# 13Karl/CUDA-Image-and-Video-codec

Measured on AMD Instinct MI355X. Metric: Mpixels/s encode (DWT+BPC) 8K P5 lossless; round-trip bit-exact, higher is better.
Workload: dtype int32

## Files before the change

### cuda-image-and-video-codec_amd/csrc/bpc_kernels.hpp

```cpp
#pragma once
#include <hip/hip_runtime.h>
#include <stdint.h>
#include <stdio.h>
#include <type_traits>

namespace picsong {

#ifdef PICSONG_DWT_TRACE
__device__ unsigned long long *g_bpc_trace = nullptr;
#define PS_BPC_TRACE(slot, val) do { if (g_bpc_trace && (threadIdx.x & 63) == 0) g_bpc_trace[(size_t)gwave * 4 + (slot)] = (val); } while (0)
#else
#define PS_BPC_TRACE(slot, val) do { } while (0)
#endif
constexpr int kMaxPlanes = 16;
constexpr int kEncPassPlanes = 8;
constexpr int kEncPlaneDwords = 4 * 64;
constexpr int kEncScratchDwordsPerWave = kMaxPlanes * kEncPlaneDwords;

struct LutGeo {
    int nBp, nSub, cRef, cSign, cSig, prec;
    int nRef, nSig, nSign;
};

constexpr int kBpcWinRects = 22;

struct BpcArgs {
    const void *coeffs_in;
    int32_t *coeffs_out;
    int is_float;
    int c16;
    int AW, AH, wl, nCB, ncx;
    int cb_base;
    const int32_t *lut;
    LutGeo g;
    int32_t *staging;
    uint16_t *staging16;
    int32_t *sizes;
    int *range_flag;
    uint32_t *plane_scratch;
    float k;
    int n_tables;
    int frames, waves_per_frame;
    unsigned long long coef_z;
    const int32_t *lut_c[3];
    const uint16_t *cw16;
    const int32_t *cw16_offsets;
    const int32_t *cw16_total;
    unsigned long long cw16_stride;
    uint32_t cw16_max;
    int ncx_r, ncb_r;
    int win_n;
    int win_x[kBpcWinRects], win_y[kBpcWinRects], win_w[kBpcWinRects], win_before[kBpcWinRects + 1];
};

__device__ __forceinline__ uint32_t from_prev32(uint32_t v, uint32_t t)
{
    uint32_t r = __builtin_amdgcn_update_dpp(0u, v, 0x138 , 0xf, 0xf, true);
    return t == 0u ? 0u : r;
}
__device__ __forceinline__ uint32_t from_next32(uint32_t v, uint32_t t)
{
    uint32_t r = __builtin_amdgcn_update_dpp(0u, v, 0x130 , 0xf, 0xf, true);
    return t == 31u ? 0u : r;
}
__device__ __forceinline__ uint32_t half_or(uint32_t v)
{
    v |= __shfl_xor(v, 16);
// ... 178 lines not shown
    const int32_t *glob;
    int total, glob_total, loff;
};
constexpr int kLutSlack = 16;
template <bool SINGLE = false>
__device__ __forceinline__ uint32_t lut_get(const LutView &v, int idx)
{
    if constexpr (SINGLE) return v.lds[idx < 0 ? 0 : (idx >= v.total ? v.total - 1 : idx)];
    return v.lds[idx];
}
template <bool SINGLE = false>
__device__ __forceinline__ PlaneLut plane_lut(const LutView &v, const LutGeo &g, int grp, int bp, int aux = 0)
{
    PlaneLut pl;
    const int ri = (grp * g.nBp + bp) * g.cRef;
    const int si = (grp * g.nBp + bp) * g.cSig + g.nRef + aux;
    const int gi = (grp * g.nBp + bp) * g.cSign + g.nRef + g.nSig + aux;
    pl.ref = lut_get<SINGLE>(v, ri);
    pl.sig0 = lut_get<SINGLE>(v, si + 0) | (lut_get<SINGLE>(v, si + 1) << 8) | (lut_get<SINGLE>(v, si + 2) << 16) | (lut_get<SINGLE>(v, si + 3) << 24);
    pl.sig1 = lut_get<SINGLE>(v, si + 4) | (lut_get<SINGLE>(v, si + 5) << 8) | (lut_get<SINGLE>(v, si + 6) << 16) | (lut_get<SINGLE>(v, si + 7) << 24);
    pl.sig8 = lut_get<SINGLE>(v, si + 8);
    pl.sign = lut_get<SINGLE>(v, gi + 0) | (lut_get<SINGLE>(v, gi + 1) << 8) | (lut_get<SINGLE>(v, gi + 2) << 16) | (lut_get<SINGLE>(v, gi + 3) << 24);
    pl.sig8x4 = pl.sig8 * 0x01010101u;
    return pl;
}
inline const char *lut_refusal(const LutGeo &g, int wl, bool bulk, bool cp3, int n_tables, char *msg, size_t cap)
{
    if (g.nBp < 1 || g.nSub < 1 || g.nRef < 1 || g.nSig < 1 || g.nSign < 1) {
        snprintf(msg, cap, "LUT geometry n_bitplanes %d, n_subbands %d, n_ref / n_sig / n_sign %d / %d / %d: every one must "
                 "be positive", g.nBp, g.nSub, g.nRef, g.nSig, g.nSign);
        return msg;
    }
    if (!bulk || cp3) {
        if (n_tables > 1) {
            snprintf(msg, cap, "LUT of %d bit-plane tables on a %s context: it codes with one table (the -k > 0 layout "
                     "belongs to a context with k > 0)", n_tables, cp3 ? "-cp 3" : "k = 0");
            return msg;
        }
        return nullptr;
    }
    const long grp_ll = (long)wl * g.nSub, grp_hh = (long)(wl - 1) * g.nSub + 2;
    const long top = (grp_ll > grp_hh ? grp_ll : grp_hh) * g.nBp + kMaxPlanes;
    const long one = (long)g.nRef + g.nSig + g.nSign;
    long reach = top * g.cRef;
    if ((long)g.nRef + top * g.cSig > reach) reach = (long)g.nRef + top * g.cSig;
    if ((long)g.nRef + g.nSig + top * g.cSign > reach) reach = (long)g.nRef + g.nSig + top * g.cSign;
// ... 641 lines not shown
    }
}


#ifndef PICSONG_BPC_PRIO
#define PICSONG_BPC_PRIO 1
#endif
__device__ __forceinline__ void prio_by_planes(int np)
{
#if PICSONG_BPC_PRIO && defined(__AMDGCN__)
    if (np >= 9) __builtin_amdgcn_s_setprio(3);
    else if (np >= 7) __builtin_amdgcn_s_setprio(2);
    else if (np >= 6) __builtin_amdgcn_s_setprio(1);
#else
    (void)np;
#endif
}

template <bool BULK, bool COMPACT = false>
__global__ __launch_bounds__(BULK ? 64 : 64 * kBpcEncWgWaves, BULK ? PICSONG_BPC_BULK_WAVES : PICSONG_BPC_ENC_WAVES) void bpc_encode_kernel(BpcArgs a)
{
    static_assert(BULK || !COMPACT, "compact table copies belong to the -k > 0 instantiations");
    constexpr int kTab = COMPACT ? kBulkCompactBytes : kLutLdsMax;
    __shared__ uint8_t lds_lut[(BULK ? 2 : 1) * kTab];
    __shared__ uint32_t lds_cnt[2 * (BULK ? 1 : kBpcEncWgWaves)];
    __shared__ uint8_t sign_tab[BULK ? 256 : 4];
    const uint32_t lane = threadIdx.x & 63u, half = lane >> 5, t = lane & 31u;
    if constexpr (BULK) sign_table2_fill(sign_tab, lane);
    if (t == 0u) lds_cnt[(threadIdx.x >> 6) * 2u + half] = half * kStageCb + kStageBytes;
    const int gwave = BULK ? (int)blockIdx.x
                           : (int)blockIdx.x * kBpcEncWgWaves + (int)__builtin_amdgcn_readfirstlane(threadIdx.x >> 6);
    int wave = gwave;
    if (a.frames > 1) {
        const int f = gwave / a.waves_per_frame;
        wave = gwave - f * a.waves_per_frame;
        if (f >= a.frames) { wave = a.waves_per_frame; }
        else {
            a.coeffs_in = (const char *)a.coeffs_in + (unsigned long long)f * a.coef_z;
            a.staging16 += (size_t)f * (size_t)a.AW * (size_t)a.AH;
            a.sizes += (size_t)f * (size_t)(a.nCB - a.cb_base);
            if (a.lut_c[0]) a.lut = f == 0 ? a.lut_c[0] : (f == 1 ? a.lut_c[1] : a.lut_c[2]);
        }
    }
    const int cb = a.cb_base + 2 * wave + (int)half;
    const bool valid = cb < a.nCB;
    const int cbx = valid ? cb % a.ncx : 0, cby = valid ? cb / a.ncx : 0;
    const size_t cbase = (size_t)(cby * 64) * (size_t)a.AW + (size_t)(cbx * 64) + 2u * t;
    const uint32_t esz = a.c16 ? 2u : 4u;
    const uint32_t cbyte = (uint32_t)cbase * esz, rstride = (uint32_t)a.AW * esz;
    uint16_t *const stw = a.staging16 + (size_t)(a.cb_base + 2 * wave) * 4096u;
    uint16_t *const st = stw + (size_t)half * 4096u;
    const uint32_t prec = (uint32_t)a.g.prec;
    const uint32_t upper_mask = opaque_mask(half ? 0xFFFFFFFFu : 0u);
    uint32_t *const pscr = a.plane_scratch + (size_t)gwave * (size_t)kEncScratchDwordsPerWave + lane;

    U64 sgL = { 0u, 0u }, sgR = { 0u, 0u };
    uint32_t ormag = 0u;
    int msb = 32, msbmax = -1;
    bool coded = false;
    PS_BPC_TRACE(0, __builtin_amdgcn_s_memrealtime());
#pragma unroll 1
    for (int pass = 0; pass < kMaxPlanes / kEncPassPlanes; pass++) {
        if (valid) {
            if (a.c16) enc_transpose_pass<2>(a, pass, cbyte, rstride, pscr, ormag, sgL, sgR);
            else if (a.is_float) enc_transpose_pass<1>(a, pass, cbyte, rstride, pscr, ormag, sgL, sgR);
            else enc_transpose_pass<0>(a, pass, cbyte, rstride, pscr, ormag, sgL, sgR);
        }
        if (pass == 0) {
            ormag = half_or_dpp(ormag, upper_mask);
            msb = ormag ? 31 - __builtin_clz(ormag) : 32;
            if (valid && msb != 32 && msb > kMaxPlanes - 1) { atomicOr(a.range_flag, 1); msb = kMaxPlanes - 1; }
            coded = valid && msb != 32;
            int mm = coded ? msb : -1;
            { int o = __shfl_xor(mm, 32); mm = mm > o ? mm : o; }
            msbmax = (int)__builtin_amdgcn_readfirstlane((uint32_t)mm);
        }
        if (msbmax < (pass + 1) * kEncPassPlanes) break;
    }

    int level, sb;
    find_subband(cbx * 64 + 2 * (int)t, cby * 64, a.AW, a.AH, a.wl, level, sb);
    const int grp = level * a.g.nSub + sb;
    int cbp = 0, loff = 0;
    BulkLane bl;
    LutGeo gl = a.g;
    int grpc = grp;
    if constexpr (BULK) { cbp = bulk_setup<COMPACT>(a, coded, msb, cbx, cby, grp, t, lds_lut + half * kTab, bl, loff, gl, grpc); bl.sgt = sign_tab; }
    else lut_to_lds(a.lut, a.g.nRef + a.g.nSig + a.g.nSign, lds_lut);
    const LutView lv = { lds_lut + (BULK ? half * kTab : 0u), a.lut, a.g.nRef + a.g.nSig + a.g.nSign,
                         (a.g.nRef + a.g.nSig + a.g.nSign) * (BULK ? a.n_tables : 1), loff };

    int np = coded ? (msb + 1 - cbp > 0 ? msb + 1 - cbp : 0) : 0;
    { int o = __shfl_xor(np, 32); np = np > o ? np : o; }
    np = (int)__builtin_amdgcn_readfirstlane((uint32_t)np);
    prio_by_planes(np);

    auto load_plane = [&](int p, U64 &bL, U64 &bR) {
        const int bp = msb - p;
        bL = U64{ 0u, 0u }; bR = U64{ 0u, 0u };
        if (coded && bp >= 0) {
            const uint32_t *q = pscr + (size_t)bp * kEncPlaneDwords;
            bL.lo = q[0]; bL.hi = q[64]; bR.lo = q[128]; bR.hi = q[192];
        }
    };

    EncCoder c;
    c.L = 0u; c.S = 0u; c.off = half * kStageCb;
    c.cnt_lo = 0u; c.cnt_hi = 0u; c.emptym = ~0ull;
    c.slot = half * kStageCb;
    c.ldscnt = &lds_cnt[(threadIdx.x >> 6) * 2u + half];
    c.slot0 = half * kStageCb + kStageBytes; c.lim = c.slot0 + kStageBytes * 4094u; c.pone = 1u << prec;
    c.stw = reinterpret_cast<char *>(stw);
    U64 AL = { 0u, 0u }, AR = { 0u, 0u };
    U64 BLn, BRn;
    load_plane(0, BLn, BRn);

    bool live = coded;
    PS_BPC_TRACE(1, __builtin_amdgcn_s_memrealtime());
    PS_BPC_TRACE(3, (unsigned long long)np);
    for (int p = 0; p < np; p++) {
        const int bp = msb - p;
        if (!BULK && p > 0) {
#if PS_ENC_LDS
            wave_lds_done();
            const uint32_t used = (*c.ldscnt - c.slot0) / kStageBytes;
#else
            const uint32_t used = half ? c.cnt_hi : c.cnt_lo;
#endif
            live = live && used < 4095u;
            if (__builtin_amdgcn_ballot_w64(live) == 0ull) break;
        }
        const bool act = live && bp >= cbp;

        PlaneLut pl = { 0u, 0u, 0u, 0u, 0u, 0u };
        if (act) pl = plane_lut<!BULK>(lv, gl, grpc, bp);

        const U64 BL = BLn, BR = BRn;
        const U64 AL2 = u_or(AL, BL), AR2 = u_or(AR, BR);
        {
            const U64 sgPL = u_prev(sgR, t), sgNL = u_next(sgL, t);
            const U64 APL = u_prev(AR, t), APL2 = u_prev(AR2, t);
            const U64 ANL = u_next(AL, t), ANL2 = u_next(AL2, t);

#pragma unroll
            for (int hw = 0; hw < 2; hw++) {
                const ColHalf cpL = make_col(up_of(APL2, hw), up_of(AL2, hw), up_of(AR2, hw), w_of(APL, hw), w_of(AR, hw),
                                             dn_of(APL, hw), dn_of(AL, hw), dn_of(AR, hw),
                                             up_of(AL2, hw), up_of(sgL, hw), dn_of(AL, hw), dn_of(sgL, hw),
                                             w_of(APL, hw), w_of(sgPL, hw), w_of(AR, hw), w_of(sgR, hw), w_of(sgL, hw));
                const ColHalf cpR = make_col(up_of(AL2, hw), up_of(AR2, hw), up_of(ANL2, hw), w_of(AL2, hw), w_of(ANL2, hw),
                                             dn_of(AL, hw), dn_of(AR, hw), dn_of(ANL, hw),
                                             up_of(AR2, hw), up_of(sgR, hw), dn_of(AR, hw), dn_of(sgR, hw),
                                             w_of(AL2, hw), w_of(sgL, hw), w_of(ANL2, hw), w_of(sgNL, hw), w_of(sgR, hw));
                const uint32_t al = act ? w_of(AL, hw) : 0xFFFFFFFFu, ar = act ? w_of(AR, hw) : 0xFFFFFFFFu;
                const uint32_t nl = w_of(BL, hw) & ~al, nr = w_of(BR, hw) & ~ar;
                uint32_t rows = wave_or32(~(al & ar));
                while (rows) {
                    const uint32_t g4 = (uint32_t)__builtin_ctz(rows) & ~3u;
// ... 964 lines not shown
```

### cuda-image-and-video-codec_amd/csrc/pack_kernels.hpp

```cpp
#pragma once
#include <hip/hip_runtime.h>
#include <stdint.h>

namespace picsong {

struct HeaderArg { uint16_t h[9]; int has; };

__host__ __device__ inline unsigned scan_threads(int n) { return n <= 16384 ? 256u : 1024u; }
__device__ __forceinline__ int32_t scan_block(int32_t sum, int32_t *s_wave, int32_t &base_out)
{
    const int tid = threadIdx.x, lane = tid & 63, wave = tid >> 6;
    int32_t inc = sum;
#pragma unroll
    for (int d = 1; d < 64; d <<= 1) {
        int32_t o = __shfl_up(inc, d);
        if (lane >= d) inc += o;
    }
    if (lane == 63) s_wave[wave] = inc;
    __syncthreads();
    int32_t base = 0;
    for (int w = 0; w < wave; w++) base += s_wave[w];
    base_out = base;
    return inc;
}
// ... 16 lines not shown
{
    __shared__ int32_t s_wave[16];
    sizes += (size_t)blockIdx.x * (size_t)n; offsets += (size_t)blockIdx.x * (size_t)n; total += blockIdx.x;
    const int tid = threadIdx.x;
    const uint32_t chunk = ((uint32_t)n + blockDim.x - 1u) / blockDim.x;
    const uint32_t b = (uint32_t)tid * chunk < (uint32_t)n ? (uint32_t)tid * chunk : (uint32_t)n, e = b + chunk < (uint32_t)n ? b + chunk : (uint32_t)n;
    int32_t sum = 0;
    uint32_t g = b;
#pragma clang loop unroll(disable) vectorize(disable) interleave(disable)
    for (; g + 8u <= e; g += 8u) {
        int32_t v[8];
        __builtin_memcpy(v, sizes + g, 32);
#pragma unroll
        for (uint32_t q = 0; q < 8u; q++) sum += v[q] - 1;
    }
#pragma clang loop unroll(disable) vectorize(disable) interleave(disable)
    for (; g < e; g++) sum += sizes[g] - 1;
    int32_t base;
    const int32_t inc = scan_block(sum, s_wave, base);
    scan_write_offsets(sizes, offsets, b, e, base + inc - sum);
    if (tid == (int)blockDim.x - 1) *total = 9 + 2 * n + (base + inc) + 1;
}

template <typename W>
__global__ __launch_bounds__(256) void pack_kernel(const W *staging, const int32_t *sizes,
                                                   const int32_t *offsets, const int32_t *total, int n,
                                                   HeaderArg hdr, uint16_t *out, size_t frame_words = 0,
                                                   size_t out_stride = 0)
{
    const int cb = blockIdx.x, tid = threadIdx.x;
    {
        const size_t f = blockIdx.y;
        staging += f * frame_words; sizes += f * (size_t)n; offsets += f * (size_t)n; total += f; out += f * out_stride;
        hdr.has = hdr.has < 0 ? (int)(((unsigned)(-hdr.has) >> f) & 1u) : ((hdr.has != 0 && (size_t)(hdr.has - 1) == f) ? 1 : 0);
    }
    const W *st = staging + (size_t)cb * 4096u;
    const int len = sizes[cb];
    uint16_t *dst = out + 9 + 2 * (size_t)n + (size_t)offsets[cb];
    if constexpr (sizeof(W) == 2) {
        const int nw = len - 1, np = (nw + 1) >> 1;
        uint32_t v[8];
        if (np > 0) {
#pragma unroll
            for (int q = 0; q < 8; q++) {
                const int pr = tid + 256 * q, pc = pr < np ? pr : np - 1;
                const int w0 = 1 + 2 * pc, wl = w0 < 4094 ? w0 : 4094;
                __builtin_memcpy(&v[q], st + wl, 4);
                if (wl != w0) v[q] >>= 16;
            }
        }
#pragma unroll
        for (int q = 0; q < 8; q++) {
            const int pr = tid + 256 * q;
            if (pr < np) {
                if (2 * pr + 1 < nw) __builtin_memcpy(dst + 2 * pr, &v[q], 4);
                else dst[2 * pr] = (uint16_t)v[q];
            }
        }
    } else {
#pragma unroll
        for (int k = 0; k < 16; k += 8) {
            if (1 + 256 * k >= len) break;
            W v[8];
#pragma unroll
            for (int q = 0; q < 8; q++) { const int j = 1 + tid + 256 * (k + q); v[q] = j < len ? st[j] : (W)0; }
#pragma unroll
            for (int q = 0; q < 8; q++) { const int j = 1 + tid + 256 * (k + q); if (j < len) dst[j - 1] = (uint16_t)v[q]; }
        }
    }
    if (tid == 0) {
        out[9 + 2 * cb] = (uint16_t)st[0];
        out[9 + 2 * cb + 1] = (uint16_t)len;
    }
    if (cb == 0) {
        if (tid < 9) out[tid] = hdr.has ? hdr.h[tid] : (uint16_t)0xFFFFu;
        if (tid == 9) out[*total - 1] = (uint16_t)0xFFFFu;
    }
}

// ... 94 lines not shown
```

### cuda-image-and-video-codec_amd/csrc/picsong_hip.hip

```cpp
#include "../../include/picsong_hip.h"

#include <hip/hip_runtime.h>

#include <cmath>
#include <cstdarg>
#include <cstdio>
#include <cstdlib>
#include <cstring>
#include <string>
#include <vector>

#include "bpc_kernels.hpp"
#include "dwt_kernels.hpp"
#include "launch_plan.hpp"
#include "window_kernels.hpp"
#include "pack_kernels.hpp"

using namespace picsong;

namespace {

thread_local char g_err[512] = "";

int fail(int code, const char *fmt, ...)
// ... 11 lines not shown
        if (e_ != hipSuccess)                                                              \
            return fail(PICSONG_ERR_HIP, "%s failed: %s (%s:%d)", #expr, hipGetErrorString(e_), \
                        __FILE__, __LINE__);                                               \
    } while (0)


}

struct picsong_ctx {
    picsong_params p;
    int device;
    int aw, ah, ncb;
    int dec_waves;
    size_t P, extra;
    bool fast_div;
    bool c16;
    bool c16_dec;
    int bulk_compact[3];
    bool pipelined;
    picsong_lut_info li[3];
    int32_t *d_lut[3];
    bool has_lut[3];
    bool lut_borrowed[3];
    int32_t *d_offsets;
    uint32_t *d_plane_scratch;
    int32_t *d_total;
    int *d_flag;
    int32_t *h_pinned;
    void *d_coef;
    int32_t *d_staging;
    int32_t *d_sizes;
    int32_t *d_coef_i;
    int batch_cap;
    void *b_coef; int32_t *b_staging, *b_sizes, *b_offsets, *b_total;
    int32_t *b_coef_i;
    int b_coef_i_cap;
    uint32_t *b_plane_scratch;
    int32_t *h_totals;
    int last_batch;
    std::vector<hipEvent_t> *prof_ev;
    int prof_cap, prof_n;
};

template <int BAND>
static void launch_inv(const picsong_ctx *c, const InvLaunch &f, hipStream_t s, unsigned frames = 1)
{
// ... 312 lines not shown
    c->bulk_compact[0] = c->bulk_compact[1] = c->bulk_compact[2] = -1;
    c->c16_dec = p->cp != 3 && p->bit_depth == 8 &&
                 dec_c16_ok(p->lossy != 0, p->wl, p->qs, p->is_rgb ? 255 : 128, c->aw, c->ah, c->fast_div);
    hipError_t e = hipMalloc(&c->d_offsets, sizeof(int32_t) * (size_t)c->ncb);
    if (e == hipSuccess) e = hipMalloc(&c->d_total, sizeof(int32_t));
    if (e == hipSuccess) e = hipMalloc(&c->d_flag, sizeof(int));
    if (e == hipSuccess) e = hipHostMalloc(&c->h_pinned, 2 * sizeof(int32_t));
    if (e == hipSuccess) e = hipMemset(c->d_flag, 0, sizeof(int));
    if (e == hipSuccess) e = hipMemset(c->d_total, 0, sizeof(int32_t));
    if (e != hipSuccess) {
        picsong_ctx_destroy(c);
        return fail(PICSONG_ERR_HIP, "ctx_create: %s", hipGetErrorString(e));
    }
    *out = c;
    return PICSONG_OK;
}

void picsong_ctx_destroy(picsong_ctx *c)
{
    if (!c) return;
    (void)hipSetDevice(c->device);
    for (int k = 0; k < 3; k++)
        if (c->d_lut[k] && !c->lut_borrowed[k]) (void)hipFree(c->d_lut[k]);
    if (c->d_offsets) (void)hipFree(c->d_offsets);
    if (c->d_plane_scratch) (void)hipFree(c->d_plane_scratch);
    if (c->d_total) (void)hipFree(c->d_total);
    if (c->d_flag) (void)hipFree(c->d_flag);
    if (c->h_pinned) (void)hipHostFree(c->h_pinned);
    if (c->d_coef) (void)hipFree(c->d_coef);
    if (c->d_staging) (void)hipFree(c->d_staging);
    if (c->d_sizes) (void)hipFree(c->d_sizes);
    if (c->d_coef_i) (void)hipFree(c->d_coef_i);
    if (c->b_coef) (void)hipFree(c->b_coef);
    if (c->b_staging) (void)hipFree(c->b_staging);
    if (c->b_sizes) (void)hipFree(c->b_sizes);
    if (c->b_offsets) (void)hipFree(c->b_offsets);
    if (c->b_total) (void)hipFree(c->b_total);
    if (c->b_plane_scratch) (void)hipFree(c->b_plane_scratch);
    if (c->b_coef_i) (void)hipFree(c->b_coef_i);
    c->b_coef_i = nullptr; c->b_coef_i_cap = 0;
    if (c->h_totals) (void)hipHostFree(c->h_totals);
    if (c->prof_ev) {
        for (hipEvent_t e : *c->prof_ev) (void)hipEventDestroy(e);
        delete c->prof_ev;
    }
    delete c;
}

static int lut_admit(const picsong_ctx *c, const picsong_lut_info &li, int n_tables)
{
    LutGeo g;
    g.nBp = li.n_bitplanes; g.nSub = li.n_subbands; g.cRef = li.ctx_ref; g.cSign = li.ctx_sign; g.cSig = li.ctx_sig;
    g.prec = li.precision; g.nRef = li.n_ref; g.nSig = li.n_sig; g.nSign = li.n_sign;
    char msg[320];
    if (lut_refusal(g, c->p.wl, c->p.k > 0.0f, c->p.cp == 3, n_tables, msg, sizeof msg))
        return fail(PICSONG_ERR_ARG, "%s", msg);
    return PICSONG_OK;
}

int picsong_ctx_set_lut_component(picsong_ctx *c, int comp, const picsong_lut_info *info, const int32_t *host_table)
{
    if (!c || !info || !host_table) return fail(PICSONG_ERR_ARG, "set_lut: null argument");
    if (comp < 0 || comp > 2) return fail(PICSONG_ERR_ARG, "set_lut: component %d outside 0..2", comp);
    if (info->ctx_sig != 9 || info->ctx_sign != 4 || info->ctx_ref != 1)
        return fail(PICSONG_ERR_ARG, "LUT contexts must be 9/4/1 (sig/sign/ref), got %d/%d/%d", info->ctx_sig,
                    info->ctx_sign, info->ctx_ref);
    if (info->precision < 1 || info->precision > 8) return fail(PICSONG_ERR_ARG, "LUT precision %d", info->precision);
    const bool cp3 = c->p.cp == 3;
    if (cp3 != (info->cp == 3))
        return fail(PICSONG_ERR_ARG, "the context codes %d passes, the table is laid out for %d (picsong_lut_load_cp)",
                    c->p.cp, info->cp == 3 ? 3 : 2);
    const size_t one = (size_t)info->n_ref + (cp3 ? 2 : 1) * ((size_t)info->n_sig + info->n_sign);
    const int n_tables = info->n_tables > 0 ? info->n_tables : 1;
    if (one + (size_t)kLutSlack > (size_t)(cp3 ? kLutLdsMax3 : kLutLdsMax))
        return fail(PICSONG_ERR_ARG, "LUT table of %zu entries exceeds the %d the coder kernels hold in LDS", one,
                    (cp3 ? kLutLdsMax3 : kLutLdsMax) - kLutSlack);
    const size_t total = one * (size_t)n_tables;
    for (size_t i = 0; i < total; i++)
        if (host_table[i] < 0 || host_table[i] > 255)
            return fail(PICSONG_ERR_ARG, "LUT entry %zu = %d outside 0..255", i, host_table[i]);
    if (int rc = lut_admit(c, *info, n_tables)) return rc;
    HIP_TRY(hipSetDevice(c->device));
    if (c->d_lut[comp] && !c->lut_borrowed[comp]) (void)hipFree(c->d_lut[comp]);
    c->d_lut[comp] = nullptr;
    c->lut_borrowed[comp] = false;
    HIP_TRY(hipMalloc(&c->d_lut[comp], total * sizeof(int32_t)));
    HIP_TRY(hipMemcpy(c->d_lut[comp], host_table, total * sizeof(int32_t), hipMemcpyHostToDevice));
    c->li[comp] = *info;
    c->li[comp].n_tables = n_tables;
    c->has_lut[comp] = true;
    c->bulk_compact[comp] = -1;
    return PICSONG_OK;
}

int picsong_ctx_set_lut_device(picsong_ctx *c, int comp, const picsong_lut_info *info, const int32_t *d_table)
{
    if (!c || !info || !d_table) return fail(PICSONG_ERR_ARG, "set_lut_device: null argument");
    if (comp < 0 || comp > 2) return fail(PICSONG_ERR_ARG, "set_lut_device: component %d outside 0..2", comp);
    if (info->ctx_sig != 9 || info->ctx_sign != 4 || info->ctx_ref != 1)
        return fail(PICSONG_ERR_ARG, "LUT contexts must be 9/4/1 (sig/sign/ref), got %d/%d/%d", info->ctx_sig,
                    info->ctx_sign, info->ctx_ref);
    if (info->precision < 1 || info->precision > 8) return fail(PICSONG_ERR_ARG, "LUT precision %d", info->precision);
    picsong_lut_info li = *info;
    const int wl = c->p.wl;
    if (li.n_ref <= 0) li.n_ref = li.n_subbands * li.n_bitplanes * li.ctx_ref * wl + li.n_bitplanes * li.ctx_ref;
    if (li.n_sig <= 0) li.n_sig = li.n_subbands * li.n_bitplanes * li.ctx_sig * wl + li.n_bitplanes * li.ctx_sig;
    if (li.n_sign <= 0) li.n_sign = li.n_subbands * li.n_bitplanes * li.ctx_sign * wl + li.n_bitplanes * li.ctx_sign;
    const bool cp3 = c->p.cp == 3;
    if (info->cp != 0 && cp3 != (info->cp == 3))
        return fail(PICSONG_ERR_ARG, "the context codes %d passes, the device table is laid out for %d", c->p.cp,
                    info->cp == 3 ? 3 : 2);
    li.cp = c->p.cp;
    const size_t one = (size_t)li.n_ref + (cp3 ? 2 : 1) * ((size_t)li.n_sig + li.n_sign);
    if (one + (size_t)kLutSlack > (size_t)(cp3 ? kLutLdsMax3 : kLutLdsMax))
        return fail(PICSONG_ERR_ARG, "LUT table of %zu entries exceeds the %d the coder kernels hold in LDS", one,
                    (cp3 ? kLutLdsMax3 : kLutLdsMax) - kLutSlack);
    if (li.n_tables <= 0) li.n_tables = 1;
    if (int rc = lut_admit(c, li, li.n_tables)) return rc;
    if (c->d_lut[comp] && !c->lut_borrowed[comp]) (void)hipFree(c->d_lut[comp]);
    c->d_lut[comp] = const_cast<int32_t *>(d_table);
    c->lut_borrowed[comp] = true;
    c->li[comp] = li;
    c->has_lut[comp] = true;
    c->bulk_compact[comp] = -1;
    return PICSONG_OK;
}

int picsong_ctx_set_lut(picsong_ctx *c, const picsong_lut_info *info, const int32_t *host_table)
{
    return picsong_ctx_set_lut_component(c, 0, info, host_table);
}

int picsong_ctx_set_pipelined(picsong_ctx *c, int on)
{
    if (!c) return fail(PICSONG_ERR_ARG, "set_pipelined: null context");
    c->pipelined = on != 0;
    return PICSONG_OK;
}

int picsong_ctx_padded_dims(const picsong_ctx *c, int *aw, int *ah, int *ncb)
{
// ... 146 lines not shown
{
    if (!c || !d_in || !d_out) return fail(PICSONG_ERR_ARG, "dwt_inverse: null argument");
    hipStream_t s = (hipStream_t)stream;
    for (const InvLaunch &f : plan_dwt_inverse(d_in, d_out, c->aw, c->ah, c->p.wl, c->p.qs, c->fast_div)) {
        switch (f.band) {
        case 32: launch_inv<32>(c, f, s); break;
        case 16: launch_inv<16>(c, f, s); break;
        case 8: launch_inv<8>(c, f, s); break;
        default: launch_inv<4>(c, f, s); break;
        }
        HIP_TRY(hipGetLastError());
    }
    return PICSONG_OK;
}

static int bpc_args(picsong_ctx *c, BpcArgs &a, int comp = 0)
{
    if (comp < 0 || comp > 2) return fail(PICSONG_ERR_ARG, "component %d outside 0..2", comp);
    if (!c->has_lut[comp]) return fail(PICSONG_ERR_ARG, "no LUT loaded for component %d: call picsong_ctx_set_lut first", comp);
    memset(&a, 0, sizeof a);
    const picsong_lut_info &li = c->li[comp];
    a.AW = c->aw; a.AH = c->ah; a.wl = c->p.wl; a.nCB = c->ncb; a.ncx = c->aw / PICSONG_CB;
    a.lut = c->d_lut[comp];
    a.g.nBp = li.n_bitplanes; a.g.nSub = li.n_subbands; a.g.cRef = li.ctx_ref;
    a.g.cSign = li.ctx_sign; a.g.cSig = li.ctx_sig; a.g.prec = li.precision;
    a.g.nRef = li.n_ref; a.g.nSig = li.n_sig; a.g.nSign = li.n_sign;
    a.range_flag = c->d_flag;
    a.k = c->p.k; a.n_tables = li.n_tables > 0 ? li.n_tables : 1;
    return PICSONG_OK;
}

static bool bulk_compact(picsong_ctx *c, int comp)
{
    if (const char *e = getenv("PICSONG_BULK_FULLTAB")) if (atoi(e) != 0) return false;
    if (c->bulk_compact[comp] < 0) {
        const picsong_lut_info &li = c->li[comp];
        c->bulk_compact[comp] = bulk_max_span_bytes(c->aw, c->ah, c->p.wl, li.n_bitplanes, li.n_subbands, li.ctx_ref, li.ctx_sig,
                                                    li.ctx_sign) <= kBulkCompactBytes ? 1 : 0;
    }
    return c->bulk_compact[comp] == 1;
}

static int dec_scratch_waves(const picsong_ctx *c) { return c->dec_waves; }
static int ensure_plane_scratch(picsong_ctx *c)
{
    static_assert(kBpcEncWgWaves == kBpcDecWgWaves, "one scratch serves the launches of both directions");
// ... 7 lines not shown
static int bpc_encode_impl(picsong_ctx *c, const void *d_coeffs, uint16_t *d_stage16, int32_t *d_sizes,
                           hipStream_t s, int cb_begin = 0, int cb_count = -1, int comp = 0, bool c16 = false)
{
    BpcArgs a;
    int rc = bpc_args(c, a, comp);
    if (rc) return rc;
    a.c16 = c16 ? 1 : 0;
    if (cb_count < 0) cb_count = c->ncb - cb_begin;
    a.cb_base = cb_begin;
    a.nCB = cb_begin + cb_count;
    a.coeffs_in = d_coeffs; a.is_float = c->p.lossy ? 1 : 0;
    a.staging16 = d_stage16; a.sizes = d_sizes;
    if (int rc2 = ensure_plane_scratch(c)) return rc2;
    a.plane_scratch = c->d_plane_scratch;
    if (c->p.cp == 3) {
        bpc3_kernel<false><<<(unsigned)(((cb_count + 1) / 2 + kBpc3WgWaves - 1) / kBpc3WgWaves), 64 * kBpc3WgWaves, 0, s>>>(a);
        HIP_TRY(hipGetLastError());
        return PICSONG_OK;
    }
    if (a.k > 0.0f) {
        if (bulk_compact(c, comp) && c->pipelined) bpc_encode_kernel<true, true><<<(unsigned)((cb_count + 1) / 2), 64, 0, s>>>(a);
        else bpc_encode_kernel<true><<<(unsigned)((cb_count + 1) / 2), 64, 0, s>>>(a);
    }
    else bpc_encode_kernel<false><<<(unsigned)(((cb_count + 1) / 2 + kBpcEncWgWaves - 1) / kBpcEncWgWaves), 64 * kBpcEncWgWaves, 0, s>>>(a);
    HIP_TRY(hipGetLastError());
    return PICSONG_OK;
}

static int bpc_encode_widened(picsong_ctx *c, const void *d_coeffs, int32_t *d_staging, int32_t *d_sizes, hipStream_t s, int comp)
{
    HIP_TRY(hipSetDevice(c->device));
    if (!c->d_staging) HIP_TRY(hipMalloc(&c->d_staging, c->P * sizeof(int32_t)));
    if (d_staging == c->d_staging) return fail(PICSONG_ERR_ARG, "bpc_encode: the context's own staging passed as the output");
    uint16_t *const st16 = reinterpret_cast<uint16_t *>(c->d_staging);
    HIP_TRY(hipMemsetAsync(d_staging, 0xFF, c->P * sizeof(int32_t), s));
    int rc = bpc_encode_impl(c, d_coeffs, st16, d_sizes, s, 0, -1, comp);
    if (rc) return rc;
    widen_staging_kernel<<<(unsigned)c->ncb, 256, 0, s>>>(st16, d_sizes, 0, d_staging);
    HIP_TRY(hipGetLastError());
    return PICSONG_OK;
}

int picsong_bpc_encode(picsong_ctx *c, const void *d_coeffs, int32_t *d_staging, int32_t *d_sizes, void *stream)
{
    if (!c || !d_coeffs || !d_staging || !d_sizes) return fail(PICSONG_ERR_ARG, "bpc_encode: null argument");
    return bpc_encode_widened(c, d_coeffs, d_staging, d_sizes, (hipStream_t)stream, 0);
}
// ... 134 lines not shown
}

int picsong_last_total(picsong_ctx *c, void *stream, int *h_total)
{
    if (!c || !h_total) return fail(PICSONG_ERR_ARG, "last_total: null argument");
    hipStream_t s = (hipStream_t)stream;
    HIP_TRY(hipMemcpyAsync(&c->h_pinned[0], c->d_total, sizeof(int32_t), hipMemcpyDeviceToHost, s));
    HIP_TRY(hipStreamSynchronize(s));
    *h_total = c->h_pinned[0];
    return PICSONG_OK;
}

extern "C++" {
template <typename W>
static int pack_range(picsong_ctx *c, const W *d_staging, const int32_t *d_sizes, int n,
                      const uint16_t *h_header, uint16_t *d_stream, hipStream_t s)
{
    HeaderArg h;
    memset(&h, 0, sizeof h);
    if (h_header) { memcpy(h.h, h_header, sizeof h.h); h.has = 1; }
    c->last_batch = 0;
    scan_sizes_kernel<<<1, scan_threads(n), 0, s>>>(d_sizes, n, c->d_offsets, c->d_total);
    HIP_TRY(hipGetLastError());
    pack_kernel<W><<<(unsigned)n, 256, 0, s>>>(d_staging, d_sizes, c->d_offsets, c->d_total, n, h, d_stream);
    HIP_TRY(hipGetLastError());
    return PICSONG_OK;
}
}

int picsong_bitstream_pack(picsong_ctx *c, const int32_t *d_staging, const int32_t *d_sizes,
                           const uint16_t *h_header, uint16_t *d_stream, int *h_total, void *stream)
{
    if (!c || !d_staging || !d_sizes || !d_stream) return fail(PICSONG_ERR_ARG, "bitstream_pack: null argument");
    int rc = pack_range(c, d_staging, d_sizes, c->ncb, h_header, d_stream, (hipStream_t)stream);
    if (rc) return rc;
    if (h_total) return picsong_last_total(c, stream, h_total);
    return PICSONG_OK;
}

static int unpack_impl(picsong_ctx *c, const uint16_t *d_stream, int32_t *d_staging, int32_t *d_sizes,
                       bool memset_staging, hipStream_t s)
{
    if (memset_staging) HIP_TRY(hipMemsetAsync(d_staging, 0xFF, c->P * sizeof(int32_t), s));
    read_sizes_kernel<<<(unsigned)((c->ncb + 255) / 256), 256, 0, s>>>(d_stream, c->ncb, d_sizes, c->d_flag);
    HIP_TRY(hipGetLastError());
    scan_sizes_kernel<<<1, scan_threads(c->ncb), 0, s>>>(d_sizes, c->ncb, c->d_offsets, c->d_total);
    HIP_TRY(hipGetLastError());
// ... 312 lines not shown
    std::vector<FwdLaunch> plan = plan_dwt_forward(d_frames, true, c->b_coef, c->aw, c->ah, c->p.wl, c->p.qs, c->c16);
    a.c16 = plan_is_c16(plan) ? 1 : 0;
    for (size_t l = 0; l < plan.size(); l++) {
        plan[l].a.src_z = l == 0 ? (unsigned long long)frame_stride : (unsigned long long)coef_z;
        plan[l].a.dst_z = (unsigned long long)coef_z;
    }
    Fwd2Launch f2;
    const bool fused01 = plan_dwt_fwd2(plan, f2, true, c->p.lossy != 0);
    if (fused01) {
        launch_fwd2(c->p.lossy != 0, f2, s, (unsigned)n);
        HIP_TRY(hipGetLastError());
    }
    if (int rc = launch_fwd_levels(c, plan, fused01 ? 2 : 0, s, (unsigned)n)) return rc;

    if (ev) HIP_TRY(hipEventRecord(ev[1], s));
    const int wpf = (c->ncb + 1) / 2;
    a.cb_base = 0; a.nCB = c->ncb;
    a.coeffs_in = c->b_coef; a.is_float = c->p.lossy ? 1 : 0;
    a.staging16 = reinterpret_cast<uint16_t *>(c->b_staging);
    a.sizes = c->b_sizes; a.plane_scratch = c->b_plane_scratch;
    a.frames = n; a.waves_per_frame = wpf; a.coef_z = coef_z;
    const size_t waves = (size_t)n * (size_t)wpf;
    if (a.k > 0.0f) launch_bulk_encode_frames(c, a, (unsigned)n, bulk_compact(c, 0), s);
    else bpc_encode_kernel<false><<<(unsigned)((waves + kBpcEncWgWaves - 1) / kBpcEncWgWaves), 64 * kBpcEncWgWaves, 0, s>>>(a);
    HIP_TRY(hipGetLastError());

    if (ev) HIP_TRY(hipEventRecord(ev[2], s));
    HeaderArg h;
    memset(&h, 0, sizeof h);
    if (first_iter <= 0 && first_iter + n > 0) {
        uint16_t hdr[PICSONG_HDR_SHORTS];
        picsong_header_pack(&c->p, hdr);
        memcpy(h.h, hdr, sizeof h.h);
        h.has = -first_iter + 1;
    }
    scan_sizes_kernel<<<(unsigned)n, scan_threads(c->ncb), 0, s>>>(c->b_sizes, c->ncb, c->b_offsets, c->b_total);
    HIP_TRY(hipGetLastError());
    pack_kernel<uint16_t><<<dim3((unsigned)c->ncb, (unsigned)n), 256, 0, s>>>(a.staging16, c->b_sizes, c->b_offsets, c->b_total,
                                                                              c->ncb, h, d_streams, c->P, stream_stride);
    HIP_TRY(hipGetLastError());
    if (ev) HIP_TRY(hipEventRecord(ev[3], s));
    c->last_batch = n;
    return PICSONG_OK;
}

int picsong_last_totals(picsong_ctx *c, void *stream, int n, int *h_totals)
{
    if (!c || !h_totals) return fail(PICSONG_ERR_ARG, "last_totals: null argument");
    if (n < 1 || n > c->last_batch) return fail(PICSONG_ERR_ARG, "last_totals: %d frames, the last batch had %d", n, c->last_batch);
    HIP_TRY(hipSetDevice(c->device));
    hipStream_t s = (hipStream_t)stream;
    HIP_TRY(hipMemcpyAsync(c->h_totals, c->b_total, (size_t)n * sizeof(int32_t), hipMemcpyDeviceToHost, s));
    HIP_TRY(hipStreamSynchronize(s));
    for (int i = 0; i < n; i++) h_totals[i] = c->h_totals[i];
    return PICSONG_OK;
}

static int decode_frames_impl(picsong_ctx *c, int n, const uint16_t *d_streams, size_t stream_stride, uint8_t *d_frames_out,
                              size_t frame_stride, void *stream, int reduce, const char *who,
                              const WindowPlan *win = nullptr, size_t pitch = 0)
{
// ... 153 lines not shown

int picsong_decode_plane(picsong_ctx *c, const uint16_t *d_stream, int comp, void *d_plane_out, void *stream)
{
    if (!c || !d_plane_out || !d_stream) return fail(PICSONG_ERR_ARG, "decode_plane: null argument");
    int rc = ensure_workspace(c, true);
    if (rc) return rc;
    hipStream_t s = (hipStream_t)stream;
    if ((rc = decode_stream_impl(c, d_stream, c->d_coef_i, s, comp))) return rc;
    return picsong_dwt_inverse(c, c->d_coef_i, d_plane_out, stream);
}


static int bpc_args_rgb(picsong_ctx *c, BpcArgs &a)
{
    int rc = bpc_args(c, a, 0);
    if (rc) return rc;
    for (int k = 1; k < 3; k++) {
        if (!c->has_lut[k]) return fail(PICSONG_ERR_ARG, "no LUT loaded for component %d", k);
        const picsong_lut_info &x = c->li[0], &y = c->li[k];
        if (x.n_bitplanes != y.n_bitplanes || x.n_subbands != y.n_subbands || x.precision != y.precision ||
            x.n_ref != y.n_ref || x.n_sig != y.n_sig || x.n_sign != y.n_sign || x.n_tables != y.n_tables)
            return fail(PICSONG_ERR_ARG, "the components' tables differ in geometry: code the planes one by one (picsong_encode_plane)");
    }
    for (int k = 0; k < 3; k++) a.lut_c[k] = c->d_lut[k];
    const int wpf = (c->ncb + 1) / 2;
    a.cb_base = 0; a.nCB = c->ncb;
    a.frames = 3; a.waves_per_frame = (wpf + kBpcEncWgWaves - 1) / kBpcEncWgWaves * kBpcEncWgWaves;
    return PICSONG_OK;
}

int picsong_encode_rgb_frame(picsong_ctx *c, const uint8_t *d_r, const uint8_t *d_g, const uint8_t *d_b, int header_mask,
                             uint16_t *d_streams, size_t stream_stride, void *stream)
{
    if (!c || !d_r || !d_g || !d_b || !d_streams) return fail(PICSONG_ERR_ARG, "encode_rgb_frame: null argument");
    if (!c->p.is_rgb) return fail(PICSONG_ERR_ARG, "encode_rgb_frame: the context is not an RGB one");
    if (c->p.cp == 3) return fail(PICSONG_ERR_ARG, "encode_rgb_frame: -cp 3 codes its planes one by one (picsong_encode_plane)");
    if (stream_stride < picsong_max_stream_shorts(c->aw, c->ah)) return fail(PICSONG_ERR_ARG, "encode_rgb_frame: stream stride smaller than a worst-case codestream");
    HIP_TRY(hipSetDevice(c->device));
    BpcArgs a;
    int rc = bpc_args_rgb(c, a);
    if (rc) return rc;
    if ((rc = ensure_batch(c, 3))) return rc;
    if ((rc = ensure_coef_i(c, 3))) return rc;
    hipStream_t s = (hipStream_t)stream;
    const size_t coef_z = (c->P + c->extra) * 4;
    char *planes = (char *)c->b_coef_i;
    bool fused_rgb = false;
// ... 12 lines not shown
            else dwt_fwd2_kernel<int, false, true, kF2PairsRgb, true, true><<<dim3(f2.gx, f2.gy, 3u), 256, 0, s>>>(f2.a);
            HIP_TRY(hipGetLastError());
            if ((rc = launch_fwd_levels(c, plan, 2, s, 3u))) return rc;
            a.c16 = 1;
            fused_rgb = true;
        }
    }
    if (!fused_rgb) {
    if ((rc = picsong_rgb_forward(c, d_r, d_g, d_b, planes, planes + c->P * 4, planes + 2 * c->P * 4, stream))) return rc;
    std::vector<FwdLaunch> plan = plan_dwt_forward(planes, false, c->b_coef, c->aw, c->ah, c->p.wl, c->p.qs, c->c16);
    a.c16 = plan_is_c16(plan) ? 1 : 0;
    for (size_t l = 0; l < plan.size(); l++) {
        plan[l].a.src_z = l == 0 ? (unsigned long long)c->P * 4ull : (unsigned long long)coef_z;
        plan[l].a.dst_z = (unsigned long long)coef_z;
    }
    if ((rc = launch_fwd_levels(c, plan, 0, s, 3u))) return rc;
    }
    a.coeffs_in = c->b_coef; a.is_float = c->p.lossy ? 1 : 0;
    a.staging16 = reinterpret_cast<uint16_t *>(c->b_staging);
    a.sizes = c->b_sizes; a.plane_scratch = c->b_plane_scratch; a.coef_z = coef_z;
    if (a.k > 0.0f) {
        launch_bulk_encode_frames(c, a, 3u, bulk_compact(c, 0) && bulk_compact(c, 1) && bulk_compact(c, 2), s);
    } else {
        bpc_encode_kernel<false><<<(unsigned)(3 * a.waves_per_frame / kBpcEncWgWaves), 64 * kBpcEncWgWaves, 0, s>>>(a);
    }
    HIP_TRY(hipGetLastError());
    HeaderArg h;
    memset(&h, 0, sizeof h);
    if (header_mask & 7) {
        uint16_t hdr[PICSONG_HDR_SHORTS];
        picsong_header_pack(&c->p, hdr);
        memcpy(h.h, hdr, sizeof h.h);
        h.has = -(header_mask & 7);
    }
    scan_sizes_kernel<<<3, scan_threads(c->ncb), 0, s>>>(c->b_sizes, c->ncb, c->b_offsets, c->b_total);
    HIP_TRY(hipGetLastError());
    pack_kernel<uint16_t><<<dim3((unsigned)c->ncb, 3u), 256, 0, s>>>(a.staging16, c->b_sizes, c->b_offsets, c->b_total, c->ncb, h,
                                                          d_streams, c->P, stream_stride);
    HIP_TRY(hipGetLastError());
    c->last_batch = 3;
    return PICSONG_OK;
}

static int decode_rgb_impl(picsong_ctx *c, const uint16_t *d_streams, size_t stream_stride, uint8_t *d_r, uint8_t *d_g,
                           uint8_t *d_b, void *stream, int reduce, const char *who, const WindowPlan *win = nullptr,
                           size_t pitch = 0)
{
    if (!c || !d_streams || !d_r || !d_g || !d_b) return fail(PICSONG_ERR_ARG, "%s: null argument", who);
    if (!c->p.is_rgb) return fail(PICSONG_ERR_ARG, "%s: the context is not an RGB one", who);
    if (c->p.cp == 3) return fail(PICSONG_ERR_ARG, "%s: -cp 3 decodes its planes one by one (picsong_decode_plane)", who);
    if (!reduce_ok(c->p.wl, reduce))
        return fail(PICSONG_ERR_ARG, "%s: reduce %d outside 0..%d (wl - 1)", who, reduce, c->p.wl - 1);
    if (stream_stride < picsong_max_stream_shorts(c->aw, c->ah)) return fail(PICSONG_ERR_ARG, "%s: stream stride smaller than a worst-case codestream", who);
    HIP_TRY(hipSetDevice(c->device));
    BpcArgs a;
    int rc = bpc_args_rgb(c, a);
    if (rc) return rc;
    const int wpf = decode_rect(c, a, reduce, win);
    if (reduce > 0 || win) a.waves_per_frame = (wpf + kBpcDecWgWaves - 1) / kBpcDecWgWaves * kBpcDecWgWaves;
    if ((rc = ensure_batch(c, 3))) return rc;
// ... 142 lines not shown
```

Measured before the change: 203,500.

## Precompute packed per-plane LUT records and pack codeblocks one per wave

For the k = 0 encode path, the per-(subband, bitplane) context probabilities are packed into 16-byte PlaneRec records. These are built once on the host, or by a small refresh kernel when the table is borrowed, and copied to LDS. Each bitplane then does one vector LDS read instead of about 18 clamped byte gathers. Separately, the 16-bit pack kernel now processes one codeblock per wave (four per block) using 16-byte overlapping chunk copies instead of one 256-thread block per codeblock. This adds extra device allocations and a refresh launch for borrowed tables, and the LDS footprint depends on a maximum of 7 wavelet levels.

```diff
diff --git a/cuda-image-and-video-codec_amd/csrc/bpc_kernels.hpp b/cuda-image-and-video-codec_amd/csrc/bpc_kernels.hpp
--- a/cuda-image-and-video-codec_amd/csrc/bpc_kernels.hpp
+++ b/cuda-image-and-video-codec_amd/csrc/bpc_kernels.hpp
@@ -23,6 +23,8 @@
 };
 
 constexpr int kBpcWinRects = 22;
+
+struct PlaneRec;
 
 struct BpcArgs {
     const void *coeffs_in;
@@ -43,6 +45,8 @@
     int frames, waves_per_frame;
     unsigned long long coef_z;
     const int32_t *lut_c[3];
+    const PlaneRec *plane_img;
+    const PlaneRec *img_c[3];
     const uint16_t *cw16;
     const int32_t *cw16_offsets;
     const int32_t *cw16_total;
@@ -267,6 +271,45 @@
     pl.sig8 = lut_get<SINGLE>(v, si + 8);
     pl.sign = lut_get<SINGLE>(v, gi + 0) | (lut_get<SINGLE>(v, gi + 1) << 8) | (lut_get<SINGLE>(v, gi + 2) << 16) | (lut_get<SINGLE>(v, gi + 3) << 24);
     pl.sig8x4 = pl.sig8 * 0x01010101u;
+    return pl;
+}
+struct alignas(16) PlaneRec { uint32_t sig0, sig1, sign, refsig8; };
+constexpr int kPlaneImgMaxWl = 7;
+constexpr int kPlaneImgMaxRecs = (3 * kPlaneImgMaxWl + 1) * kMaxPlanes;
+__host__ __device__ inline int plane_img_recs(int wl) { return (3 * wl + 1) * kMaxPlanes; }
+__host__ __device__ inline PlaneRec plane_record(const int32_t *lut, const LutGeo &g, int slot, int bp)
+{
+    const int total = g.nRef + g.nSig + g.nSign;
+    const int grp = (slot / 3) * g.nSub + slot % 3;
+    const int ri = (grp * g.nBp + bp) * g.cRef;
+    const int si = (grp * g.nBp + bp) * g.cSig + g.nRef;
+    const int gi = (grp * g.nBp + bp) * g.cSign + g.nRef + g.nSig;
+    auto at = [&](int idx) -> uint32_t { return (uint32_t)lut[idx < 0 ? 0 : (idx >= total ? total - 1 : idx)] & 0xFFu; };
+    PlaneRec r;
+    r.sig0 = at(si + 0) | (at(si + 1) << 8) | (at(si + 2) << 16) | (at(si + 3) << 24);
+    r.sig1 = at(si + 4) | (at(si + 5) << 8) | (at(si + 6) << 16) | (at(si + 7) << 24);
+    r.sign = at(gi + 0) | (at(gi + 1) << 8) | (at(gi + 2) << 16) | (at(gi + 3) << 24);
+    r.refsig8 = at(ri) | (at(si + 8) << 8);
+    return r;
+}
+__global__ __launch_bounds__(256) void plane_img_kernel(const int32_t *lut, LutGeo g, int wl, PlaneRec *img)
+{
+    for (int i = (int)threadIdx.x; i < plane_img_recs(wl); i += (int)blockDim.x) img[i] = plane_record(lut, g, i / kMaxPlanes, i % kMaxPlanes);
+}
+__device__ __forceinline__ void plane_img_to_lds(const PlaneRec *img, const int32_t *lut, const LutGeo &g, int wl, PlaneRec *lds)
+{
+    const int n = plane_img_recs(wl);
+    if (img) { for (int i = (int)threadIdx.x; i < n; i += (int)blockDim.x) lds[i] = img[i]; }
+    else { for (int i = (int)threadIdx.x; i < n; i += (int)blockDim.x) lds[i] = plane_record(lut, g, i / kMaxPlanes, i % kMaxPlanes); }
+    __syncthreads();
+}
+__device__ __forceinline__ PlaneLut plane_lut_img(const PlaneRec *lds, int slot, int bp)
+{
+    const PlaneRec r = lds[slot * kMaxPlanes + bp];
+    PlaneLut pl;
+    pl.sig0 = r.sig0; pl.sig1 = r.sig1; pl.sign = r.sign;
+    pl.ref = r.refsig8 & 0xFFu; pl.sig8 = r.refsig8 >> 8;
+    pl.sig8x4 = __builtin_amdgcn_perm(r.refsig8, r.refsig8, 0x01010101u);
     return pl;
 }
 inline const char *lut_refusal(const LutGeo &g, int wl, bool bulk, bool cp3, int n_tables, char *msg, size_t cap)
@@ -954,7 +997,7 @@
 {
     static_assert(BULK || !COMPACT, "compact table copies belong to the -k > 0 instantiations");
     constexpr int kTab = COMPACT ? kBulkCompactBytes : kLutLdsMax;
-    __shared__ uint8_t lds_lut[(BULK ? 2 : 1) * kTab];
+    __shared__ alignas(16) uint8_t lds_lut[BULK ? 2 * kTab : kPlaneImgMaxRecs * (int)sizeof(PlaneRec)];
     __shared__ uint32_t lds_cnt[2 * (BULK ? 1 : kBpcEncWgWaves)];
     __shared__ uint8_t sign_tab[BULK ? 256 : 4];
     const uint32_t lane = threadIdx.x & 63u, half = lane >> 5, t = lane & 31u;
@@ -971,7 +1014,10 @@
             a.coeffs_in = (const char *)a.coeffs_in + (unsigned long long)f * a.coef_z;
             a.staging16 += (size_t)f * (size_t)a.AW * (size_t)a.AH;
             a.sizes += (size_t)f * (size_t)(a.nCB - a.cb_base);
-            if (a.lut_c[0]) a.lut = f == 0 ? a.lut_c[0] : (f == 1 ? a.lut_c[1] : a.lut_c[2]);
+            if (a.lut_c[0]) {
+                a.lut = f == 0 ? a.lut_c[0] : (f == 1 ? a.lut_c[1] : a.lut_c[2]);
+                a.plane_img = f == 0 ? a.img_c[0] : (f == 1 ? a.img_c[1] : a.img_c[2]);
+            }
         }
     }
     const int cb = a.cb_base + 2 * wave + (int)half;
@@ -1018,9 +1064,10 @@
     LutGeo gl = a.g;
     int grpc = grp;
     if constexpr (BULK) { cbp = bulk_setup<COMPACT>(a, coded, msb, cbx, cby, grp, t, lds_lut + half * kTab, bl, loff, gl, grpc); bl.sgt = sign_tab; }
-    else lut_to_lds(a.lut, a.g.nRef + a.g.nSig + a.g.nSign, lds_lut);
+    else plane_img_to_lds(a.plane_img, a.lut, a.g, a.wl, reinterpret_cast<PlaneRec *>(lds_lut));
     const LutView lv = { lds_lut + (BULK ? half * kTab : 0u), a.lut, a.g.nRef + a.g.nSig + a.g.nSign,
                          (a.g.nRef + a.g.nSig + a.g.nSign) * (BULK ? a.n_tables : 1), loff };
+    const PlaneRec *const recs = reinterpret_cast<const PlaneRec *>(lds_lut) + (level * 3 + sb) * kMaxPlanes;
 
     int np = coded ? (msb + 1 - cbp > 0 ? msb + 1 - cbp : 0) : 0;
     { int o = __shfl_xor(np, 32); np = np > o ? np : o; }
@@ -1065,7 +1112,7 @@
         const bool act = live && bp >= cbp;
 
         PlaneLut pl = { 0u, 0u, 0u, 0u, 0u, 0u };
-        if (act) pl = plane_lut<!BULK>(lv, gl, grpc, bp);
+        if (act) { if constexpr (BULK) pl = plane_lut<false>(lv, gl, grpc, bp); else pl = plane_lut_img(recs, 0, bp); }
 
         const U64 BL = BLn, BR = BRn;
         const U64 AL2 = u_or(AL, BL), AR2 = u_or(AR, BR);
diff --git a/cuda-image-and-video-codec_amd/csrc/pack_kernels.hpp b/cuda-image-and-video-codec_amd/csrc/pack_kernels.hpp
--- a/cuda-image-and-video-codec_amd/csrc/pack_kernels.hpp
+++ b/cuda-image-and-video-codec_amd/csrc/pack_kernels.hpp
@@ -62,13 +62,18 @@
     if (tid == (int)blockDim.x - 1) *total = 9 + 2 * n + (base + inc) + 1;
 }
 
+constexpr int kPack16Waves = 4;
+template <typename W>
+__host__ __device__ inline unsigned pack_blocks(int n) { return sizeof(W) == 2 ? (unsigned)((n + kPack16Waves - 1) / kPack16Waves) : (unsigned)n; }
 template <typename W>
 __global__ __launch_bounds__(256) void pack_kernel(const W *staging, const int32_t *sizes,
                                                    const int32_t *offsets, const int32_t *total, int n,
                                                    HeaderArg hdr, uint16_t *out, size_t frame_words = 0,
                                                    size_t out_stride = 0)
 {
-    const int cb = blockIdx.x, tid = threadIdx.x;
+    const int tid = sizeof(W) == 2 ? (int)(threadIdx.x & 63u) : (int)threadIdx.x;
+    const int cb = sizeof(W) == 2 ? (int)blockIdx.x * kPack16Waves + (int)__builtin_amdgcn_readfirstlane(threadIdx.x >> 6) : (int)blockIdx.x;
+    if (cb >= n) return;
     {
         const size_t f = blockIdx.y;
         staging += f * frame_words; sizes += f * (size_t)n; offsets += f * (size_t)n; total += f; out += f * out_stride;
@@ -78,23 +83,26 @@
     const int len = sizes[cb];
     uint16_t *dst = out + 9 + 2 * (size_t)n + (size_t)offsets[cb];
     if constexpr (sizeof(W) == 2) {
-        const int nw = len - 1, np = (nw + 1) >> 1;
-        uint32_t v[8];
-        if (np > 0) {
-#pragma unroll
-            for (int q = 0; q < 8; q++) {
-                const int pr = tid + 256 * q, pc = pr < np ? pr : np - 1;
-                const int w0 = 1 + 2 * pc, wl = w0 < 4094 ? w0 : 4094;
-                __builtin_memcpy(&v[q], st + wl, 4);
-                if (wl != w0) v[q] >>= 16;
-            }
-        }
-#pragma unroll
-        for (int q = 0; q < 8; q++) {
-            const int pr = tid + 256 * q;
-            if (pr < np) {
-                if (2 * pr + 1 < nw) __builtin_memcpy(dst + 2 * pr, &v[q], 4);
-                else dst[2 * pr] = (uint16_t)v[q];
+        const uint32_t nw = len < 1 ? 0u : (len > 4096 ? 4095u : (uint32_t)(len - 1));
+        const char *const src = reinterpret_cast<const char *>(st + 1);
+        char *const dstb = reinterpret_cast<char *>(dst);
+        if (nw < 8u) {
+            const uint16_t tv = st[1u + ((uint32_t)tid < nw ? (uint32_t)tid : 0u)];
+            if ((uint32_t)tid < nw) dst[tid] = tv;
+        } else {
+            const uint32_t nch = (nw + 7u) >> 3, last = 2u * nw - 16u;
+            auto chunk_at = [&](uint32_t ci) { return 16u * ci < last ? 16u * ci : last; };
+            auto load_chunk = [&](uint32_t ci) { uint4 r; __builtin_memcpy(&r, src + chunk_at(ci), 16); return r; };
+            auto store_chunk = [&](uint32_t ci, const uint4 &r) { if (ci < nch) __builtin_memcpy(dstb + chunk_at(ci), &r, 16); };
+#pragma clang loop unroll(disable)
+            for (uint32_t c0 = 0; c0 < nch; c0 += 256u) {
+                const uint32_t ci = c0 + (uint32_t)tid;
+                uint4 v0 = load_chunk(ci);
+                const uint4 v1 = load_chunk(ci + 64u), v2 = load_chunk(ci + 128u), v3 = load_chunk(ci + 192u);
+#if defined(__AMDGCN__)
+                asm volatile("" : "+v"(v0.x));
+#endif
+                store_chunk(ci, v0); store_chunk(ci + 64u, v1); store_chunk(ci + 128u, v2); store_chunk(ci + 192u, v3);
             }
         }
     } else {
diff --git a/cuda-image-and-video-codec_amd/csrc/picsong_hip.hip b/cuda-image-and-video-codec_amd/csrc/picsong_hip.hip
--- a/cuda-image-and-video-codec_amd/csrc/picsong_hip.hip
+++ b/cuda-image-and-video-codec_amd/csrc/picsong_hip.hip
@@ -57,6 +57,7 @@
     int32_t *d_lut[3];
     bool has_lut[3];
     bool lut_borrowed[3];
+    PlaneRec *d_img[3];
     int32_t *d_offsets;
     uint32_t *d_plane_scratch;
     int32_t *d_total;
@@ -415,6 +416,8 @@
     (void)hipSetDevice(c->device);
     for (int k = 0; k < 3; k++)
         if (c->d_lut[k] && !c->lut_borrowed[k]) (void)hipFree(c->d_lut[k]);
+    for (int k = 0; k < 3; k++)
+        if (c->d_img[k]) (void)hipFree(c->d_img[k]);
     if (c->d_offsets) (void)hipFree(c->d_offsets);
     if (c->d_plane_scratch) (void)hipFree(c->d_plane_scratch);
     if (c->d_total) (void)hipFree(c->d_total);
@@ -451,6 +454,37 @@
     return PICSONG_OK;
 }
 
+static bool ctx_uses_plane_img(const picsong_ctx *c) { return !(c->p.k > 0.0f) && c->p.cp != 3; }
+static LutGeo lut_geo(const picsong_lut_info &li)
+{
+    LutGeo g;
+    g.nBp = li.n_bitplanes; g.nSub = li.n_subbands; g.cRef = li.ctx_ref; g.cSign = li.ctx_sign; g.cSig = li.ctx_sig;
+    g.prec = li.precision; g.nRef = li.n_ref; g.nSig = li.n_sig; g.nSign = li.n_sign;
+    return g;
+}
+static int plane_img_alloc(picsong_ctx *c, int comp)
+{
+    if (!c->d_img[comp]) HIP_TRY(hipMalloc(&c->d_img[comp], kPlaneImgMaxRecs * sizeof(PlaneRec)));
+    return PICSONG_OK;
+}
+static int plane_img_from_host(picsong_ctx *c, int comp, const picsong_lut_info &li, const int32_t *host_table)
+{
+    if (!ctx_uses_plane_img(c)) return PICSONG_OK;
+    if (int rc = plane_img_alloc(c, comp)) return rc;
+    const LutGeo g = lut_geo(li);
+    std::vector<PlaneRec> img((size_t)plane_img_recs(c->p.wl));
+    for (size_t i = 0; i < img.size(); i++) img[i] = plane_record(host_table, g, (int)i / kMaxPlanes, (int)i % kMaxPlanes);
+    HIP_TRY(hipMemcpy(c->d_img[comp], img.data(), img.size() * sizeof(PlaneRec), hipMemcpyHostToDevice));
+    return PICSONG_OK;
+}
+static int plane_img_refresh(picsong_ctx *c, int comp, hipStream_t s)
+{
+    if (!ctx_uses_plane_img(c) || !c->lut_borrowed[comp]) return PICSONG_OK;
+    plane_img_kernel<<<1, 256, 0, s>>>(c->d_lut[comp], lut_geo(c->li[comp]), c->p.wl, c->d_img[comp]);
+    HIP_TRY(hipGetLastError());
+    return PICSONG_OK;
+}
+
 int picsong_ctx_set_lut_component(picsong_ctx *c, int comp, const picsong_lut_info *info, const int32_t *host_table)
 {
     if (!c || !info || !host_table) return fail(PICSONG_ERR_ARG, "set_lut: null argument");
@@ -474,6 +508,7 @@
             return fail(PICSONG_ERR_ARG, "LUT entry %zu = %d outside 0..255", i, host_table[i]);
     if (int rc = lut_admit(c, *info, n_tables)) return rc;
     HIP_TRY(hipSetDevice(c->device));
+    if (int rc = plane_img_from_host(c, comp, *info, host_table)) return rc;
     if (c->d_lut[comp] && !c->lut_borrowed[comp]) (void)hipFree(c->d_lut[comp]);
     c->d_lut[comp] = nullptr;
     c->lut_borrowed[comp] = false;
@@ -510,6 +545,10 @@
                     (cp3 ? kLutLdsMax3 : kLutLdsMax) - kLutSlack);
     if (li.n_tables <= 0) li.n_tables = 1;
     if (int rc = lut_admit(c, li, li.n_tables)) return rc;
+    if (ctx_uses_plane_img(c)) {
+        HIP_TRY(hipSetDevice(c->device));
+        if (int rc = plane_img_alloc(c, comp)) return rc;
+    }
     if (c->d_lut[comp] && !c->lut_borrowed[comp]) (void)hipFree(c->d_lut[comp]);
     c->d_lut[comp] = const_cast<int32_t *>(d_table);
     c->lut_borrowed[comp] = true;
@@ -702,6 +741,7 @@
     const picsong_lut_info &li = c->li[comp];
     a.AW = c->aw; a.AH = c->ah; a.wl = c->p.wl; a.nCB = c->ncb; a.ncx = c->aw / PICSONG_CB;
     a.lut = c->d_lut[comp];
+    a.plane_img = ctx_uses_plane_img(c) ? c->d_img[comp] : nullptr;
     a.g.nBp = li.n_bitplanes; a.g.nSub = li.n_subbands; a.g.cRef = li.ctx_ref;
     a.g.cSign = li.ctx_sign; a.g.cSig = li.ctx_sig; a.g.prec = li.precision;
     a.g.nRef = li.n_ref; a.g.nSig = li.n_sig; a.g.nSign = li.n_sign;
@@ -755,7 +795,10 @@
         if (bulk_compact(c, comp) && c->pipelined) bpc_encode_kernel<true, true><<<(unsigned)((cb_count + 1) / 2), 64, 0, s>>>(a);
         else bpc_encode_kernel<true><<<(unsigned)((cb_count + 1) / 2), 64, 0, s>>>(a);
     }
-    else bpc_encode_kernel<false><<<(unsigned)(((cb_count + 1) / 2 + kBpcEncWgWaves - 1) / kBpcEncWgWaves), 64 * kBpcEncWgWaves, 0, s>>>(a);
+    else {
+        if (int rc2 = plane_img_refresh(c, comp, s)) return rc2;
+        bpc_encode_kernel<false><<<(unsigned)(((cb_count + 1) / 2 + kBpcEncWgWaves - 1) / kBpcEncWgWaves), 64 * kBpcEncWgWaves, 0, s>>>(a);
+    }
     HIP_TRY(hipGetLastError());
     return PICSONG_OK;
 }
@@ -936,7 +979,7 @@
     c->last_batch = 0;
     scan_sizes_kernel<<<1, scan_threads(n), 0, s>>>(d_sizes, n, c->d_offsets, c->d_total);
     HIP_TRY(hipGetLastError());
-    pack_kernel<W><<<(unsigned)n, 256, 0, s>>>(d_staging, d_sizes, c->d_offsets, c->d_total, n, h, d_stream);
+    pack_kernel<W><<<pack_blocks<W>(n), 256, 0, s>>>(d_staging, d_sizes, c->d_offsets, c->d_total, n, h, d_stream);
     HIP_TRY(hipGetLastError());
     return PICSONG_OK;
 }
@@ -1295,7 +1338,10 @@
     a.frames = n; a.waves_per_frame = wpf; a.coef_z = coef_z;
     const size_t waves = (size_t)n * (size_t)wpf;
     if (a.k > 0.0f) launch_bulk_encode_frames(c, a, (unsigned)n, bulk_compact(c, 0), s);
-    else bpc_encode_kernel<false><<<(unsigned)((waves + kBpcEncWgWaves - 1) / kBpcEncWgWaves), 64 * kBpcEncWgWaves, 0, s>>>(a);
+    else {
+        if ((rc = plane_img_refresh(c, 0, s))) return rc;
+        bpc_encode_kernel<false><<<(unsigned)((waves + kBpcEncWgWaves - 1) / kBpcEncWgWaves), 64 * kBpcEncWgWaves, 0, s>>>(a);
+    }
     HIP_TRY(hipGetLastError());
 
     if (ev) HIP_TRY(hipEventRecord(ev[2], s));
@@ -1309,7 +1355,7 @@
     }
     scan_sizes_kernel<<<(unsigned)n, scan_threads(c->ncb), 0, s>>>(c->b_sizes, c->ncb, c->b_offsets, c->b_total);
     HIP_TRY(hipGetLastError());
-    pack_kernel<uint16_t><<<dim3((unsigned)c->ncb, (unsigned)n), 256, 0, s>>>(a.staging16, c->b_sizes, c->b_offsets, c->b_total,
+    pack_kernel<uint16_t><<<dim3(pack_blocks<uint16_t>(c->ncb), (unsigned)n), 256, 0, s>>>(a.staging16, c->b_sizes, c->b_offsets, c->b_total,
                                                                               c->ncb, h, d_streams, c->P, stream_stride);
     HIP_TRY(hipGetLastError());
     if (ev) HIP_TRY(hipEventRecord(ev[3], s));
@@ -1509,7 +1555,7 @@
             x.n_ref != y.n_ref || x.n_sig != y.n_sig || x.n_sign != y.n_sign || x.n_tables != y.n_tables)
             return fail(PICSONG_ERR_ARG, "the components' tables differ in geometry: code the planes one by one (picsong_encode_plane)");
     }
-    for (int k = 0; k < 3; k++) a.lut_c[k] = c->d_lut[k];
+    for (int k = 0; k < 3; k++) { a.lut_c[k] = c->d_lut[k]; a.img_c[k] = ctx_uses_plane_img(c) ? c->d_img[k] : nullptr; }
     const int wpf = (c->ncb + 1) / 2;
     a.cb_base = 0; a.nCB = c->ncb;
     a.frames = 3; a.waves_per_frame = (wpf + kBpcEncWgWaves - 1) / kBpcEncWgWaves * kBpcEncWgWaves;
@@ -1568,6 +1614,7 @@
     if (a.k > 0.0f) {
         launch_bulk_encode_frames(c, a, 3u, bulk_compact(c, 0) && bulk_compact(c, 1) && bulk_compact(c, 2), s);
     } else {
+        for (int k = 0; k < 3; k++) if ((rc = plane_img_refresh(c, k, s))) return rc;
         bpc_encode_kernel<false><<<(unsigned)(3 * a.waves_per_frame / kBpcEncWgWaves), 64 * kBpcEncWgWaves, 0, s>>>(a);
     }
     HIP_TRY(hipGetLastError());
@@ -1581,7 +1628,7 @@
     }
     scan_sizes_kernel<<<3, scan_threads(c->ncb), 0, s>>>(c->b_sizes, c->ncb, c->b_offsets, c->b_total);
     HIP_TRY(hipGetLastError());
-    pack_kernel<uint16_t><<<dim3((unsigned)c->ncb, 3u), 256, 0, s>>>(a.staging16, c->b_sizes, c->b_offsets, c->b_total, c->ncb, h,
+    pack_kernel<uint16_t><<<dim3(pack_blocks<uint16_t>(c->ncb), 3u), 256, 0, s>>>(a.staging16, c->b_sizes, c->b_offsets, c->b_total, c->ncb, h,
                                                           d_streams, c->P, stream_stride);
     HIP_TRY(hipGetLastError());
     c->last_batch = 3;
```

New measurement: 208,500, median of 6. 2.5% higher.
